# NEUROINFORMATICS-GROUP-FAV-KIV-ZCU/EEG_DataAnalysisPackage

Measured on AMD Instinct MI355X. Metric: epochs/sec feature-extracted (whole node) + % HBM roofline, 1/2/4/8 GPUs, higher is better.
Workload: dtype f64

## Files before the change

eeg_dataanalysispackage_amd/csrc/logreg.hip:

```cpp
#include <hip/hip_runtime.h>

#include <cstdint>
#include <cstdlib>

#include "launch.h"

namespace eegfx {
namespace dev {

constexpr int kLrWaves = 4;
#ifndef EEGFX_LR_UNROLL
#define EEGFX_LR_UNROLL 4
#endif

__device__ __forceinline__ double wave_sum(double v) {
#pragma unroll
  for (int off = 32; off > 0; off >>= 1) v += __shfl_xor(v, off, 64);
  return v;
}

template <int GRAD>
__device__ __forceinline__ double grad_mult(double margin, double y) {
  if constexpr (GRAD == 0) {
    return 1.0 / (1.0 + exp(-margin)) - y;
  } else {
    const double s = 2.0 * y - 1.0;
    return 1.0 > s * margin ? -s : 0.0;
  }
}

template <int GRAD>
__device__ __forceinline__ double axpy_row(double mult, double x, double acc) {
  if constexpr (GRAD == 0) {
    return __builtin_fma(mult, x, acc);
  } else {
    return mult != 0.0 ? __builtin_fma(mult, x, acc) : acc;
  }
}

__device__ __forceinline__ bool sampled(const uint32_t* __restrict__ mask, int64_t r) {
  return !mask || ((mask[r >> 5] >> (r & 31)) & 1u);
}

template <int KD, int GRAD>
__global__ __launch_bounds__(64 * kLrWaves) void lr_grad_kernel(
    const double* __restrict__ X, const double* __restrict__ y, int64_t n, int d,
    const uint32_t* __restrict__ mask, const LrState* __restrict__ st,
    double* __restrict__ partial) {
  if (st->converged) return;
  __shared__ double acc_s[kLrWaves][64 * KD];
  const int lane = threadIdx.x & 63, w = threadIdx.x >> 6;
  const double* wt = st->w;
  double wv[KD], acc[KD];
#pragma unroll
  for (int k = 0; k < KD; ++k) {
    const int f = lane + 64 * k;
    wv[k] = f < d ? wt[f] : 0.0;
    acc[k] = 0.0;
  }
  const int64_t stride = (int64_t)gridDim.x * kLrWaves;
  for (int64_t r = (int64_t)blockIdx.x * kLrWaves + w; r < n; r += stride) {
    if (!sampled(mask, r)) continue;
    const double* row = X + r * d;
    double x[KD];
    double dot = 0.0;
#pragma unroll
    for (int k = 0; k < KD; ++k) {
      const int f = lane + 64 * k;
      x[k] = f < d ? row[f] : 0.0;
      dot = __builtin_fma(x[k], wv[k], dot);
    }
    dot = wave_sum(dot);
    const double mult = grad_mult<GRAD>(dot, y[r]);
#pragma unroll
    for (int k = 0; k < KD; ++k) acc[k] = axpy_row<GRAD>(mult, x[k], acc[k]);
  }
#pragma unroll
  for (int k = 0; k < KD; ++k) acc_s[w][lane + 64 * k] = acc[k];
  __syncthreads();
  for (int f = threadIdx.x; f < d; f += blockDim.x) {
    double s = acc_s[0][f];
#pragma unroll
    for (int v = 1; v < kLrWaves; ++v) s += acc_s[v][f];
    partial[(int64_t)blockIdx.x * d + f] = s;
  }
}

template <int CTRL>
__device__ __forceinline__ double dpp_d(double v) {
  const uint64_t u = __builtin_bit_cast(uint64_t, v);
  const int lo = __builtin_amdgcn_update_dpp(0, (int)(uint32_t)u, CTRL, 0xF, 0xF, false);
  const int hi = __builtin_amdgcn_update_dpp(0, (int)(uint32_t)(u >> 32), CTRL, 0xF, 0xF, false);
  return __builtin_bit_cast(double, ((uint64_t)(uint32_t)hi << 32) | (uint32_t)lo);
}
__device__ __forceinline__ double row16_sum(double v) {
  v += dpp_d<0xB1>(v);
  v += dpp_d<0x4E>(v);
  v += dpp_d<0x141>(v);
  v += dpp_d<0x140>(v);
  return v;
}

template <int FPL, int GRAD>
__global__ __launch_bounds__(64 * kLrWaves) void lr_grad16_kernel(
    const double* __restrict__ X, const double* __restrict__ y, int64_t n, int d,
    const uint32_t* __restrict__ mask, const LrState* __restrict__ st,
    double* __restrict__ partial) {
  if (st->converged) return;
  __shared__ double acc_s[kLrWaves * 4][16 * FPL];
  const int lane = threadIdx.x & 63, w = threadIdx.x >> 6;
  const int q = lane >> 4, j = lane & 15;
  double wv[FPL], acc[FPL];
#pragma unroll
  for (int k = 0; k < FPL; ++k) {
    const int f = j + 16 * k;
    wv[k] = f < d ? st->w[f] : 0.0;
    acc[k] = 0.0;
  }
  constexpr int U = EEGFX_LR_UNROLL;
  const int64_t stride = (int64_t)gridDim.x * kLrWaves * 4 * U;
  for (int64_t r0 = ((int64_t)blockIdx.x * kLrWaves + w) * 4 * U; r0 < n; r0 += stride) {
    double x[U][FPL], dot[U], yy[U];
#pragma unroll
    for (int u = 0; u < U; ++u) {
      const int64_t r = r0 + 4 * u + q;
      dot[u] = 0.0;
      if constexpr (GRAD == 0) {
        const bool ok = r < n && sampled(mask, r);
        const double* row = X + (ok ? r : 0) * d;
#pragma unroll
        for (int k = 0; k < FPL; ++k) {
          const int f = j + 16 * k;
          x[u][k] = (ok && f < d) ? row[f] : 0.0;
          dot[u] = __builtin_fma(x[u][k], wv[k], dot[u]);
        }
        yy[u] = ok ? y[r] : 0.0;
      } else {
        const double* row = X + (r < n ? r : n - 1) * d;
#pragma unroll
        for (int k = 0; k < FPL; ++k) {
          const int f = j + 16 * k;
          x[u][k] = row[f < d ? f : d - 1];
          dot[u] = __builtin_fma(x[u][k], wv[k], dot[u]);
        }
        yy[u] = y[r < n ? r : n - 1];
      }
    }
    double mult[U], msum = 0.0;
#pragma unroll
    for (int u = 0; u < U; ++u) {
      const double m = row16_sum(dot[u]);
      const bool ok = r0 + 4 * u + q < n && sampled(mask, r0 + 4 * u + q);
      mult[u] = ok ? grad_mult<GRAD>(m, yy[u]) : 0.0;
      msum += m;
    }
    if constexpr (GRAD == 1) {
      if (__builtin_amdgcn_ballot_w64(!(__builtin_fabs(msum) <= __DBL_MAX__)) != 0) {
#pragma unroll
        for (int u = 0; u < U; ++u) {
          double dt = 0.0;
#pragma unroll
          for (int k = 0; k < FPL; ++k) {
            if (j + 16 * k >= d) x[u][k] = 0.0;
            dt = __builtin_fma(x[u][k], wv[k], dt);
          }
          const double m = row16_sum(dt);
          const bool ok = r0 + 4 * u + q < n && sampled(mask, r0 + 4 * u + q);
          const double mu = ok ? grad_mult<GRAD>(m, yy[u]) : 0.0;
#pragma unroll
          for (int k = 0; k < FPL; ++k) acc[k] = axpy_row<GRAD>(mu, x[u][k], acc[k]);
        }
        continue;
      }
    }
#pragma unroll
    for (int u = 0; u < U; ++u) {
#pragma unroll
      for (int k = 0; k < FPL; ++k) acc[k] = __builtin_fma(mult[u], x[u][k], acc[k]);
    }
  }
#pragma unroll
  for (int k = 0; k < FPL; ++k) acc_s[w * 4 + q][j + 16 * k] = acc[k];
  __syncthreads();
  for (int f = threadIdx.x; f < d; f += blockDim.x) {
    double s = acc_s[0][f];
#pragma unroll
    for (int v = 1; v < kLrWaves * 4; ++v) s += acc_s[v][f];
    partial[(int64_t)blockIdx.x * d + f] = s;
  }
}

__global__ __launch_bounds__(256) void lr_update_kernel(const double* __restrict__ partial, int G,
                                                        int64_t n, int d, double step_size,
                                                        double reg, double tol, int max_iter,
                                                        LrState* __restrict__ st) {
  if (st->converged) return;
  __shared__ double red[2][256];
  __shared__ double gs[256];
  const int it = st->iter + 1;
  const double step = step_size / sqrt((double)it);
  const int K = d <= 128 ? (int)blockDim.x / d : 1;
  if (K > 1) {
    const int t = threadIdx.x, jj = t / d, f = t - jj * d;
    if (jj < K) {
      double a0 = 0.0, a1 = 0.0;
      int b = jj;
      for (; b + K < G; b += 2 * K) {
        a0 += partial[(int64_t)b * d + f];
        a1 += partial[(int64_t)(b + K) * d + f];
      }
      if (b < G) a0 += partial[(int64_t)b * d + f];
      gs[t] = a0 + a1;
    }
    __syncthreads();
  }
  double diff2 = 0.0, norm2 = 0.0;
  for (int f = threadIdx.x; f < d; f += blockDim.x) {
    double g = 0.0;
    if (K > 1) {
      for (int jj = 0; jj < K; ++jj) g += gs[jj * d + f];
    } else {
      for (int b = 0; b < G; ++b) g += partial[(int64_t)b * d + f];
    }
    g = g / (double)n;
    const double old = st->w[f];
    double nw = old * (1.0 - step * reg);
    nw = nw + (-step) * g;
    st->w[f] = nw;
    diff2 += (old - nw) * (old - nw);
    norm2 += nw * nw;
  }
  red[0][threadIdx.x] = diff2;
  red[1][threadIdx.x] = norm2;
  __syncthreads();
  for (int s = 128; s > 0; s >>= 1) {
    if ((int)threadIdx.x < s) {
      red[0][threadIdx.x] += red[0][threadIdx.x + s];
      red[1][threadIdx.x] += red[1][threadIdx.x + s];
    }
    __syncthreads();
  }
  if (threadIdx.x == 0) {
    st->iter = it;
    const int up = st->updates + 1;
    st->updates = up;
    const double diff = sqrt(red[0][0]), nrm = sqrt(red[1][0]);
    if ((up >= 2 && diff < tol * (nrm > 1.0 ? nrm : 1.0)) || it >= max_iter) st->converged = 1;
  }
}

__global__ void lr_skip_kernel(int max_iter, LrState* __restrict__ st) {
  if (st->converged || threadIdx.x != 0) return;
  st->iter += 1;
  if (st->iter >= max_iter) st->converged = 1;
}

template <int KD, int KIND>
__global__ __launch_bounds__(256) void lr_predict_kernel(const double* __restrict__ X, int64_t n,
                                                         int d, const double* __restrict__ wt,
                                                         double intercept, double threshold,
                                                         int use_threshold,
                                                         double* __restrict__ out) {
  const int lane = threadIdx.x & 63;
  const int64_t r = (int64_t)blockIdx.x * 4 + (threadIdx.x >> 6);
  if (r >= n) return;
  double dot = 0.0;
#pragma unroll
  for (int k = 0; k < KD; ++k) {
    const int f = lane + 64 * k;
    if (f < d) dot = __builtin_fma(X[r * d + f], wt[f], dot);
  }
  dot = wave_sum(dot);
  if (lane == 0) {
    const double margin = dot + intercept;
    const double score = KIND == 0 ? 1.0 / (1.0 + exp(-margin)) : margin;
    out[r] = use_threshold ? (score > threshold ? 1.0 : 0.0) : score;
  }
}

__global__ __launch_bounds__(256) void lr_validate_kernel(const double* __restrict__ y, int64_t n,
                                                          LrState* __restrict__ st) {
  for (int64_t i = (int64_t)blockIdx.x * blockDim.x + threadIdx.x; i < n;
       i += (int64_t)gridDim.x * blockDim.x)
    if (!(y[i] == 0.0 || y[i] == 1.0)) st->converged = 2;
}

}

hipError_t launch_lr_validate(hipStream_t st, const double* y, int64_t n, LrState* state) {
  const int64_t g = (n + 255) / 256;
  hipLaunchKernelGGL(dev::lr_validate_kernel, dim3((unsigned)(g < 1 ? 1 : (g > 4096 ? 4096 : g))),
                     dim3(256), 0, st, y, n, state);
  return hipGetLastError();
}

int lr_grid(int64_t n) {
  constexpr int64_t cap = 512;
  const int64_t g = (n + 16 * dev::kLrWaves - 1) / (16 * dev::kLrWaves);
  return (int)(g < 1 ? 1 : (g > cap ? cap : g));
}

#define EEGFX_LR_KD(KD, CALL) \
  case KD:                    \
    CALL;                     \
    break;

template <int GRAD>
static hipError_t lr_iteration(hipStream_t st, const double* X, const double* y, int64_t n, int d,
                               const uint32_t* mask, int64_t count, LrState* state,
                               double* partial, int G, double step_size, double reg, double tol,
                               int max_iter) {
  if (count == 0) {
    hipLaunchKernelGGL(dev::lr_skip_kernel, dim3(1), dim3(64), 0, st, max_iter, state);
    return hipGetLastError();
  }
  if (d <= 128) {
    const int fpl = (d + 15) / 16;
    switch (fpl <= 1 ? 1 : fpl <= 2 ? 2 : fpl <= 3 ? 3 : fpl <= 4 ? 4 : 8) {
      EEGFX_LR_KD(1, hipLaunchKernelGGL((dev::lr_grad16_kernel<1, GRAD>), dim3(G), dim3(256), 0,
                                        st, X, y, n, d, mask, state, partial))
      EEGFX_LR_KD(2, hipLaunchKernelGGL((dev::lr_grad16_kernel<2, GRAD>), dim3(G), dim3(256), 0,
                                        st, X, y, n, d, mask, state, partial))
      EEGFX_LR_KD(3, hipLaunchKernelGGL((dev::lr_grad16_kernel<3, GRAD>), dim3(G), dim3(256), 0,
                                        st, X, y, n, d, mask, state, partial))
      EEGFX_LR_KD(4, hipLaunchKernelGGL((dev::lr_grad16_kernel<4, GRAD>), dim3(G), dim3(256), 0,
                                        st, X, y, n, d, mask, state, partial))
      EEGFX_LR_KD(8, hipLaunchKernelGGL((dev::lr_grad16_kernel<8, GRAD>), dim3(G), dim3(256), 0,
                                        st, X, y, n, d, mask, state, partial))
    }
  } else {
    const int kd = (d + 63) / 64;
    switch (kd <= 1 ? 1 : kd <= 2 ? 2 : kd <= 4 ? 4 : kd <= 8 ? 8 : 16) {
      EEGFX_LR_KD(1, hipLaunchKernelGGL((dev::lr_grad_kernel<1, GRAD>), dim3(G), dim3(256), 0, st,
                                        X, y, n, d, mask, state, partial))
      EEGFX_LR_KD(2, hipLaunchKernelGGL((dev::lr_grad_kernel<2, GRAD>), dim3(G), dim3(256), 0, st,
                                        X, y, n, d, mask, state, partial))
      EEGFX_LR_KD(4, hipLaunchKernelGGL((dev::lr_grad_kernel<4, GRAD>), dim3(G), dim3(256), 0, st,
                                        X, y, n, d, mask, state, partial))
      EEGFX_LR_KD(8, hipLaunchKernelGGL((dev::lr_grad_kernel<8, GRAD>), dim3(G), dim3(256), 0, st,
                                        X, y, n, d, mask, state, partial))
      EEGFX_LR_KD(16, hipLaunchKernelGGL((dev::lr_grad_kernel<16, GRAD>), dim3(G), dim3(256), 0,
                                         st, X, y, n, d, mask, state, partial))
    }
  }
  hipLaunchKernelGGL(dev::lr_update_kernel, dim3(1), dim3(256), 0, st, partial, G, count, d,
                     step_size, reg, tol, max_iter, state);
  return hipGetLastError();
}

hipError_t launch_lr_iteration(hipStream_t st, int grad, const double* X, const double* y,
                               int64_t n, int d, const uint32_t* mask, int64_t count,
                               LrState* state, double* partial, int G, double step_size,
                               double reg, double tol, int max_iter) {
  return grad == kGradHinge ? lr_iteration<1>(st, X, y, n, d, mask, count, state, partial, G,
                                              step_size, reg, tol, max_iter)
                            : lr_iteration<0>(st, X, y, n, d, mask, count, state, partial, G,
                                              step_size, reg, tol, max_iter);
}

template <int KIND>
static hipError_t lr_predict(hipStream_t st, const double* X, int64_t n, int d, const double* w,
                             double intercept, double threshold, int use_threshold, double* out) {
  const dim3 grid((unsigned)((n + 3) / 4));
  const int kd = (d + 63) / 64;
  switch (kd <= 1 ? 1 : kd <= 2 ? 2 : kd <= 4 ? 4 : kd <= 8 ? 8 : 16) {
    EEGFX_LR_KD(1, hipLaunchKernelGGL((dev::lr_predict_kernel<1, KIND>), grid, dim3(256), 0, st, X,
                                      n, d, w, intercept, threshold, use_threshold, out))
    EEGFX_LR_KD(2, hipLaunchKernelGGL((dev::lr_predict_kernel<2, KIND>), grid, dim3(256), 0, st, X,
                                      n, d, w, intercept, threshold, use_threshold, out))
    EEGFX_LR_KD(4, hipLaunchKernelGGL((dev::lr_predict_kernel<4, KIND>), grid, dim3(256), 0, st, X,
                                      n, d, w, intercept, threshold, use_threshold, out))
    EEGFX_LR_KD(8, hipLaunchKernelGGL((dev::lr_predict_kernel<8, KIND>), grid, dim3(256), 0, st, X,
                                      n, d, w, intercept, threshold, use_threshold, out))
    EEGFX_LR_KD(16, hipLaunchKernelGGL((dev::lr_predict_kernel<16, KIND>), grid, dim3(256), 0, st,
                                       X, n, d, w, intercept, threshold, use_threshold, out))
  }
  return hipGetLastError();
}

hipError_t launch_lr_predict(hipStream_t st, int grad, const double* X, int64_t n, int d,
                             const double* w, double intercept, double threshold,
                             int use_threshold, double* out) {
  if (n == 0) return hipSuccess;
  return grad == kGradHinge
             ? lr_predict<1>(st, X, n, d, w, intercept, threshold, use_threshold, out)
             : lr_predict<0>(st, X, n, d, w, intercept, threshold, use_threshold, out);
}
#undef EEGFX_LR_KD

}
```

Before: 1.165 billion.

## Software-pipeline logreg gradient row loads and batch partial-sum loads in update

Restructures the gradient kernel loop into a two-stage software pipeline that prefetches the next stride's rows and labels into registers while computing the current one. Mask bits are fetched once per 32-row group instead of per row, and groups with no sampled rows are skipped. The update kernel now issues 32 independent partial loads before accumulating, which adds memory-level parallelism. Costs are higher register pressure, from the doubled x buffers and the 32-wide load batch, which may reduce occupancy.

```diff
diff --git a/eeg_dataanalysispackage_amd/csrc/logreg.hip b/eeg_dataanalysispackage_amd/csrc/logreg.hip
--- a/eeg_dataanalysispackage_amd/csrc/logreg.hip
+++ b/eeg_dataanalysispackage_amd/csrc/logreg.hip
@@ -9,6 +9,7 @@
 namespace dev {
 
 constexpr int kLrWaves = 4;
+constexpr int kLrBatch = 32;
 #ifndef EEGFX_LR_UNROLL
 #define EEGFX_LR_UNROLL 4
 #endif
@@ -102,6 +103,108 @@
 }
 
 template <int FPL, int GRAD>
+struct LrGroup {
+  static constexpr int U = EEGFX_LR_UNROLL;
+  static constexpr bool kAhead = GRAD == 0 && FPL <= 4;
+  static_assert(32 % (4 * U) == 0, "a group's sample bits lie in one mask word");
+  const double* __restrict__ X;
+  const double* __restrict__ y;
+  const uint32_t* __restrict__ mask;
+  int64_t n;
+  int d, q, j;
+
+  __device__ __forceinline__ uint32_t bits(int64_t g0) const {
+    const int64_t c = g0 < n ? g0 : n - 1;
+    uint32_t b = ~0u;
+    if (mask) b = mask[c >> 5] >> (int)(c & 31);
+    const int64_t left = n - g0;
+    const int rows = left >= 4 * U ? 4 * U : left > 0 ? (int)left : 0;
+    return rows == 32 ? b : b & ((1u << rows) - 1u);
+  }
+  __device__ __forceinline__ void load(int64_t g0, uint32_t b, int u, double (&xu)[FPL],
+                                       double& yu) const {
+    const int64_t r = g0 + 4 * u + q;
+    int64_t rc;
+    if constexpr (GRAD == 0) rc = ((b >> (4 * u + q)) & 1u) ? r : 0;
+    else rc = r < n ? r : n - 1;
+    const double* row = X + rc * d;
+#pragma unroll
+    for (int k = 0; k < FPL; ++k) {
+      const int f = j + 16 * k;
+      xu[k] = row[f < d ? f : d - 1];
+    }
+    yu = y[rc];
+  }
+};
+
+template <int FPL, int GRAD>
+__device__ __forceinline__ void lr_grad16_trip(
+    const LrGroup<FPL, GRAD>& g, int64_t r0, int64_t stride, uint32_t b, uint32_t nb,
+    double (&xc)[LrGroup<FPL, GRAD>::U][FPL], double (&yc)[LrGroup<FPL, GRAD>::U],
+    double (&xn)[LrGroup<FPL, GRAD>::U][FPL], double (&yn)[LrGroup<FPL, GRAD>::U],
+    const double (&wv)[FPL], double (&acc)[FPL]) {
+  constexpr int U = LrGroup<FPL, GRAD>::U;
+  if constexpr (!LrGroup<FPL, GRAD>::kAhead) {
+    if (b == 0) return;
+#pragma unroll
+    for (int u = 0; u < U; ++u) g.load(r0, b, u, xc[u], yc[u]);
+  } else {
+#pragma unroll
+    for (int u = 0; u < U; ++u) g.load(r0 + stride, nb, u, xn[u], yn[u]);
+    __builtin_amdgcn_sched_barrier(0);
+#pragma unroll
+    for (int u = 0; u < U; ++u) asm volatile("" : "+v"(yc[u]));
+    if (b == 0) return;
+  }
+  double x[U][FPL], dot[U], yy[U];
+  bool ok[U];
+#pragma unroll
+  for (int u = 0; u < U; ++u) {
+    ok[u] = (b >> (4 * u + g.q)) & 1u;
+    dot[u] = 0.0;
+#pragma unroll
+    for (int k = 0; k < FPL; ++k) {
+      const double v = xc[u][k];
+      if constexpr (GRAD == 0) x[u][k] = (ok[u] && g.j + 16 * k < g.d) ? v : 0.0;
+      else x[u][k] = v;
+      dot[u] = __builtin_fma(x[u][k], wv[k], dot[u]);
+    }
+    if constexpr (GRAD == 0) yy[u] = ok[u] ? yc[u] : 0.0;
+    else yy[u] = yc[u];
+  }
+  double mult[U], msum = 0.0;
+#pragma unroll
+  for (int u = 0; u < U; ++u) {
+    const double m = row16_sum(dot[u]);
+    mult[u] = ok[u] ? grad_mult<GRAD>(m, yy[u]) : 0.0;
+    msum += m;
+  }
+  if constexpr (GRAD == 1) {
+    if (__builtin_amdgcn_ballot_w64(!(__builtin_fabs(msum) <= __DBL_MAX__)) != 0) {
+#pragma unroll
+      for (int u = 0; u < U; ++u) {
+        double dt = 0.0;
+#pragma unroll
+        for (int k = 0; k < FPL; ++k) {
+          if (g.j + 16 * k >= g.d) x[u][k] = 0.0;
+          dt = __builtin_fma(x[u][k], wv[k], dt);
+        }
+        const double m = row16_sum(dt);
+        const double mu = ok[u] ? grad_mult<GRAD>(m, yy[u]) : 0.0;
+#pragma unroll
+        for (int k = 0; k < FPL; ++k) acc[k] = axpy_row<GRAD>(mu, x[u][k], acc[k]);
+      }
+      return;
+    }
+  }
+#pragma unroll
+  for (int u = 0; u < U; ++u) {
+#pragma unroll
+    for (int k = 0; k < FPL; ++k) acc[k] = __builtin_fma(mult[u], x[u][k], acc[k]);
+  }
+}
+
+template <int FPL, int GRAD>
 __global__ __launch_bounds__(64 * kLrWaves) void lr_grad16_kernel(
     const double* __restrict__ X, const double* __restrict__ y, int64_t n, int d,
     const uint32_t* __restrict__ mask, const LrState* __restrict__ st,
@@ -117,66 +220,24 @@
     wv[k] = f < d ? st->w[f] : 0.0;
     acc[k] = 0.0;
   }
-  constexpr int U = EEGFX_LR_UNROLL;
+  using Group = LrGroup<FPL, GRAD>;
+  constexpr int U = Group::U;
+  const Group g{X, y, mask, n, d, q, j};
   const int64_t stride = (int64_t)gridDim.x * kLrWaves * 4 * U;
-  for (int64_t r0 = ((int64_t)blockIdx.x * kLrWaves + w) * 4 * U; r0 < n; r0 += stride) {
-    double x[U][FPL], dot[U], yy[U];
-#pragma unroll
-    for (int u = 0; u < U; ++u) {
-      const int64_t r = r0 + 4 * u + q;
-      dot[u] = 0.0;
-      if constexpr (GRAD == 0) {
-        const bool ok = r < n && sampled(mask, r);
-        const double* row = X + (ok ? r : 0) * d;
-#pragma unroll
-        for (int k = 0; k < FPL; ++k) {
-          const int f = j + 16 * k;
-          x[u][k] = (ok && f < d) ? row[f] : 0.0;
-          dot[u] = __builtin_fma(x[u][k], wv[k], dot[u]);
-        }
-        yy[u] = ok ? y[r] : 0.0;
-      } else {
-        const double* row = X + (r < n ? r : n - 1) * d;
-#pragma unroll
-        for (int k = 0; k < FPL; ++k) {
-          const int f = j + 16 * k;
-          x[u][k] = row[f < d ? f : d - 1];
-          dot[u] = __builtin_fma(x[u][k], wv[k], dot[u]);
-        }
-        yy[u] = y[r < n ? r : n - 1];
-      }
-    }
-    double mult[U], msum = 0.0;
-#pragma unroll
-    for (int u = 0; u < U; ++u) {
-      const double m = row16_sum(dot[u]);
-      const bool ok = r0 + 4 * u + q < n && sampled(mask, r0 + 4 * u + q);
-      mult[u] = ok ? grad_mult<GRAD>(m, yy[u]) : 0.0;
-      msum += m;
-    }
-    if constexpr (GRAD == 1) {
-      if (__builtin_amdgcn_ballot_w64(!(__builtin_fabs(msum) <= __DBL_MAX__)) != 0) {
-#pragma unroll
-        for (int u = 0; u < U; ++u) {
-          double dt = 0.0;
-#pragma unroll
-          for (int k = 0; k < FPL; ++k) {
-            if (j + 16 * k >= d) x[u][k] = 0.0;
-            dt = __builtin_fma(x[u][k], wv[k], dt);
-          }
-          const double m = row16_sum(dt);
-          const bool ok = r0 + 4 * u + q < n && sampled(mask, r0 + 4 * u + q);
-          const double mu = ok ? grad_mult<GRAD>(m, yy[u]) : 0.0;
-#pragma unroll
-          for (int k = 0; k < FPL; ++k) acc[k] = axpy_row<GRAD>(mu, x[u][k], acc[k]);
-        }
-        continue;
-      }
-    }
-#pragma unroll
-    for (int u = 0; u < U; ++u) {
-#pragma unroll
-      for (int k = 0; k < FPL; ++k) acc[k] = __builtin_fma(mult[u], x[u][k], acc[k]);
+  int64_t r0 = ((int64_t)blockIdx.x * kLrWaves + __builtin_amdgcn_readfirstlane(w)) * 4 * U;
+  uint32_t b0 = g.bits(r0), b1 = g.bits(r0 + stride);
+  double xa[U][FPL], ya[U], xb[U][FPL], yb[U];
+  if (r0 < n) {
+    if constexpr (Group::kAhead) {
+#pragma unroll
+      for (int u = 0; u < U; ++u) g.load(r0, b0, u, xa[u], ya[u]);
+    }
+    for (; r0 < n; r0 += 2 * stride) {
+      const uint32_t b2 = g.bits(r0 + 2 * stride), b3 = g.bits(r0 + 3 * stride);
+      lr_grad16_trip<FPL, GRAD>(g, r0, stride, b0, b1, xa, ya, xb, yb, wv, acc);
+      lr_grad16_trip<FPL, GRAD>(g, r0 + stride, stride, b1, b2, xb, yb, xa, ya, wv, acc);
+      b0 = b2;
+      b1 = b3;
     }
   }
 #pragma unroll
@@ -204,12 +265,20 @@
     const int t = threadIdx.x, jj = t / d, f = t - jj * d;
     if (jj < K) {
       double a0 = 0.0, a1 = 0.0;
-      int b = jj;
-      for (; b + K < G; b += 2 * K) {
-        a0 += partial[(int64_t)b * d + f];
-        a1 += partial[(int64_t)(b + K) * d + f];
+      for (int b = jj; b < G; b += kLrBatch * K) {
+        double v[kLrBatch];
+#pragma unroll
+        for (int i = 0; i < kLrBatch; ++i) {
+          const int bi = b + i * K;
+          v[i] = partial[(int64_t)(bi < G ? bi : b) * d + f];
+        }
+        __builtin_amdgcn_sched_barrier(0);
+#pragma unroll
+        for (int i = 0; i < kLrBatch; i += 2) {
+          if (b + i * K < G) a0 += v[i];
+          if (b + (i + 1) * K < G) a1 += v[i + 1];
+        }
       }
-      if (b < G) a0 += partial[(int64_t)b * d + f];
       gs[t] = a0 + a1;
     }
     __syncthreads();
@@ -220,7 +289,16 @@
     if (K > 1) {
       for (int jj = 0; jj < K; ++jj) g += gs[jj * d + f];
     } else {
-      for (int b = 0; b < G; ++b) g += partial[(int64_t)b * d + f];
+      for (int b = 0; b < G; b += kLrBatch) {
+        double v[kLrBatch];
+#pragma unroll
+        for (int i = 0; i < kLrBatch; ++i)
+          v[i] = partial[(int64_t)(b + i < G ? b + i : b) * d + f];
+        __builtin_amdgcn_sched_barrier(0);
+#pragma unroll
+        for (int i = 0; i < kLrBatch; ++i)
+          if (b + i < G) g += v[i];
+      }
     }
     g = g / (double)n;
     const double old = st->w[f];
```

Measured after the change: 1.170 billion, median of 4. Within noise of the previous version (+0.5%).
